# openai/procgen

Measured on NVIDIA H100. Metric: env-steps/sec, higher is better.
Workload: dtype f32+u8

## Files before the change

procgen_b200/csrc/pg_launch.cuh:

```cuda
#pragma once
#include <stdarg.h>
#include <stddef.h>
#include <stdio.h>
#include <stdlib.h>
#include <string.h>

#include <type_traits>

#include "pg_kernels.cuh"

#ifndef PG_HOSTSIM
#include <cuda_runtime.h>
#endif

namespace pg {

static inline void pg_fatal(const char *fmt, ...) {
    fprintf(stderr, "fatal: ");
    va_list args;
    va_start(args, fmt);
    vfprintf(stderr, fmt, args);
    va_end(args);
    exit(EXIT_FAILURE);
}
#define pg_fassert(cond)                                                                  \
    do {                                                                                  \
        if (!(cond)) {                                                                    \
            fprintf(stderr, "fassert failed '%s' at %s:%d\n", #cond, __FILE__, __LINE__); \
            exit(EXIT_FAILURE);                                                           \
        }                                                                                 \
    } while (0)

#ifndef PG_HOSTSIM
#define CUDA_CHECK(expr)                                                                          \
    do {                                                                                          \
        cudaError_t _e = (expr);                                                                  \
        if (_e != cudaSuccess)                                                                    \
            pg_fatal("CUDA error %s at %s:%d: %s\n", cudaGetErrorName(_e), __FILE__, __LINE__, cudaGetErrorString(_e)); \
    } while (0)
using Stream = cudaStream_t;
using Event = cudaEvent_t;
#else
struct HostStream;
struct HostEvent;
using Stream = HostStream *;
using Event = HostEvent *;
#endif

#ifndef PG_LOGIC_WARPS
#define PG_LOGIC_WARPS 2
#endif
#ifndef PG_LOGIC_MIN_BLOCKS
#define PG_LOGIC_MIN_BLOCKS 24
#endif
#ifndef PG_STEP_CHUNKS
#define PG_STEP_CHUNKS 8
#endif
#ifndef PG_AUX_STREAMS
#define PG_AUX_STREAMS 16
#endif
constexpr int kLogicThreads = 32 * PG_LOGIC_WARPS;
constexpr int kLogicEnvsPerBlock = PG_LOGIC_WARPS;
constexpr int kRenderThreads = 128;

#ifndef PG_HOSTSIM
template <class G, bool INIT, bool LEVEL_CHOICE = false, bool FINAL = false, bool PAUSE = false>
__global__ void __launch_bounds__(kLogicThreads, PG_LOGIC_MIN_BLOCKS) logic_kernel(KParams p, unsigned int *ticket) {
    using Frame = typename FrameFor<G>::type;
    const unsigned lane = threadIdx.x & 31u;
    while (true) {
        unsigned t = 0;
        if (lane == 0)
            t = atomicAdd(ticket, 1u);
        t = __shfl_sync(0xffffffffu, t, 0);
        if (t >= (unsigned)p.env_count)
            break;
        const int env = p.env_first + (int)t * p.env_step;
        const long long t0 = p.dbg_cycles ? clock64() : 0;
        env_logic<G, Frame, INIT, LEVEL_CHOICE, FINAL, PAUSE>(p, env);
        __syncwarp();
        if (p.dbg_cycles && lane == 0)
            p.dbg_cycles[env] = (uint32_t)(clock64() - t0);
    }
}

template <class G, bool BANK = false, bool LOOK = false>
__global__ void __launch_bounds__(kLogicThreads, PG_LOGIC_MIN_BLOCKS) finish_kernel(KParams p, unsigned int *ticket) {
    using Frame = typename FrameFor<G>::type;
    const unsigned lane = threadIdx.x & 31u;
    const unsigned count = *p.reset_count;
    while (true) {
        unsigned t = 0;
        if (lane == 0)
            t = atomicAdd(ticket, 1u);
        t = __shfl_sync(0xffffffffu, t, 0);
        if (t >= count)
            break;
        const int env = p.reset_list[t];
        const long long t0 = ((BANK || LOOK) && p.dbg_cycles) ? clock64() : 0;
        env_finish_logic<G, Frame, BANK, LOOK>(p, env);
        __syncwarp();
        if ((BANK || LOOK) && p.dbg_cycles && lane == 0)
            p.dbg_cycles[env] += (uint32_t)(clock64() - t0);
    }
}

template <class G>
__global__ void __launch_bounds__(kLogicThreads) bank_build_kernel(KParams p, unsigned char *stage, int count, int warps) {
    const int w = (int)((blockIdx.x * blockDim.x + threadIdx.x) >> 5);
    if (w >= warps)
        return;
    for (int item = w; item < count; item += warps) {
        bank_generate_level<G>(p, p.bank, p.bank.seeds[item], [&] { return p.bank.slots + (size_t)item * p.bank.slot_bytes; },
                               stage + (size_t)w * bank_stage_bytes(p));
        __syncwarp();
    }
}

template <class G>
__global__ void __launch_bounds__(kLogicThreads) lookahead_kernel(KParams p, unsigned int *count) {
    const int w = (int)((blockIdx.x * blockDim.x + threadIdx.x) >> 5);
    if (w >= p.look.stage_warps)
        return;
    const unsigned lane = threadIdx.x & 31u;
    const unsigned n = count[0];
    unsigned char *stage = p.look.stage + (size_t)w * bank_stage_bytes(p);
    while (true) {
        unsigned t = 0;
        if (lane == 0)
            t = atomicAdd(count + 1, 1u);
        t = __shfl_sync(0xffffffffu, t, 0);
        if (t >= n)
            break;
        lookahead_generate<G>(p, (int)t, stage);
        __syncwarp();
    }
}

template <class G>
__global__ void __launch_bounds__(kLogicThreads) lookahead_predict_kernel(KParams p) {
    const int i = (int)((blockIdx.x * blockDim.x + threadIdx.x) >> 5);
    if (i < p.env_count)
        lookahead_predict(p, p.env_first + i * p.env_step, p.bank.slots != nullptr);
}

constexpr int kSetupThreads = 128;
#ifndef PG_SETUP_MIN_BLOCKS
#define PG_SETUP_MIN_BLOCKS 8
#endif
template <class G, int VIEW>
struct SetupTune {
    static constexpr int kSmemBytes = (int)sizeof(typename FrameFor<G, VIEW>::setup) * (kSetupThreads / 32);
    static constexpr int kFit = (227 * 1024) / (kSmemBytes + 1024 + 128);
    static constexpr int kMinBlocks = kFit >= PG_SETUP_MIN_BLOCKS ? PG_SETUP_MIN_BLOCKS : (kFit >= 1 ? kFit : 1);
};
template <class G, int VIEW, bool LIST = false, bool PAUSE = false>
__global__ void __launch_bounds__(kSetupThreads, SetupTune<G, VIEW>::kMinBlocks) setup_kernel(KParams p) {
    using Setup = typename FrameFor<G, VIEW>::setup;
    extern __shared__ __align__(128) unsigned char smem_raw[];
    Setup &f = reinterpret_cast<Setup *>(smem_raw)[threadIdx.x >> 5];
    const int lane = (int)(threadIdx.x & 31u);
    const int i = (int)blockIdx.x * (kSetupThreads / 32) + (int)(threadIdx.x >> 5);
    if (LIST) {
        const int count = (int)*p.reset_count;
        for (int j = i; j < count; j += (int)gridDim.x * (kSetupThreads / 32)) {
            const int env = p.reset_list[j];
            env_setup_frame<G, Setup>(p, env, f, lane, 32);
            __syncwarp();
            PG_SETUP_PHASE_BEGIN;
            env_store_frame<Setup>(p, env, f);
            PG_SETUP_PHASE(9);
        }
        return;
    }
    if (i >= p.env_count)
        return;
    const int env = p.env_first + i * p.env_step;
    if (PAUSE && p.paused[env])
        return;
    env_setup_frame<G, Setup>(p, env, f, lane, 32);
    __syncwarp();
    PG_SETUP_PHASE_BEGIN;
    env_store_frame<Setup>(p, env, f);
    PG_SETUP_PHASE(9);
}

#ifndef PG_RENDER_CTAS_PER_SM
#define PG_RENDER_CTAS_PER_SM 0
#endif
template <class G, int VIEW>
struct RenderTune {
    static constexpr size_t kFrameBytes = sizeof(typename FrameFor<G, VIEW>::type);
#ifdef PG_RENDER_MIN_BLOCKS
    static constexpr int kMinBlocks = PG_RENDER_MIN_BLOCKS;
#else
    static constexpr int kFit = (int)((227 * 1024) / (kFrameBytes + 1024 + 16));
    static constexpr int kWant = G::DRAWS_GRID ? 7 : 8;
    static constexpr int kMinBlocks = kFit >= kWant ? kWant : (kFit >= 1 ? kFit : 1);
#endif
};

__device__ __forceinline__ uint32_t pg_smem_addr(const void *ptr) { return (uint32_t)__cvta_generic_to_shared(ptr); }
__device__ __forceinline__ void pg_mbar_init(unsigned long long *bar, unsigned count) {
    asm volatile("mbarrier.init.shared::cta.b64 [%0], %1;" ::"r"(pg_smem_addr(bar)), "r"(count) : "memory");
    asm volatile("fence.mbarrier_init.release.cluster;" ::: "memory");
}
__device__ __forceinline__ void pg_mbar_arrive_expect_tx(unsigned long long *bar, unsigned bytes) {
    asm volatile("mbarrier.arrive.expect_tx.shared::cta.b64 _, [%0], %1;" ::"r"(pg_smem_addr(bar)), "r"(bytes) : "memory");
}
__device__ __forceinline__ void pg_mbar_wait(unsigned long long *bar, unsigned parity) {
    unsigned done = 0;
    while (!done) {
        asm volatile(
            "{\n"
            ".reg .pred p;\n"
            "mbarrier.try_wait.parity.shared::cta.b64 p, [%1], %2;\n"
            "selp.u32 %0, 1, 0, p;\n"
            "}\n"
            : "=r"(done)
            : "r"(pg_smem_addr(bar)), "r"(parity)
            : "memory");
    }
}
__device__ __forceinline__ void pg_bulk_load(void *dst_smem, const void *src_gmem, unsigned bytes, unsigned long long *bar) {
    asm volatile("cp.async.bulk.shared::cluster.global.mbarrier::complete_tx::bytes [%0], [%1], %2, [%3];" ::"r"(pg_smem_addr(dst_smem)),
                 "l"(src_gmem), "r"(bytes), "r"(pg_smem_addr(bar))
                 : "memory");
}
__device__ __forceinline__ void pg_bulk_store(void *dst_gmem, const void *src_smem, unsigned bytes) {
    asm volatile("cp.async.bulk.global.shared::cta.bulk_group [%0], [%1], %2;" ::"l"(dst_gmem), "r"(pg_smem_addr(src_smem)), "r"(bytes) : "memory");
}
__device__ __forceinline__ void pg_bulk_commit_and_wait() {
    asm volatile("cp.async.bulk.commit_group;" ::: "memory");
    asm volatile("cp.async.bulk.wait_group.read 0;" ::: "memory");
}

template <class G, int VIEW, int PASS, bool ROLL, class EnvOf>
__device__ __forceinline__ void render_env_frame(const KParams &p, typename FrameFor<G, VIEW>::type &f, EnvOf env_of, unsigned parity) {
    using Frame = typename FrameFor<G, VIEW>::type;
    const int tid = (int)threadIdx.x;
#ifdef PG_PHASE_TIMING
    long long t0 = clock64(), t1;
#define PG_RENDER_PHASE(id)                                       \
    do {                                                          \
        t1 = clock64();                                           \
        if (tid == 0)                                             \
            p.hdr[env_of()].dbg_phase[id] = (uint32_t)(t1 - t0);       \
        t0 = t1;                                                  \
    } while (0)
#else
#define PG_RENDER_PHASE(id) do { } while (0)
#endif
    using Shared = typename FrameFor<G, VIEW>::shared;
    const Shared *gs = reinterpret_cast<const Shared *>(p.frame_setup + (size_t)env_of() * p.frame_setup_stride);
    if (tid < 32) {
        const int nj = G::DRAWS_GRID ? (gs->n_tjobs < MAX_TILE_JOBS ? gs->n_tjobs : MAX_TILE_JOBS) : 0;
        unsigned words = 0;
        for (int j = tid; j < nj; j += 32) words += gs->tjob_words[j];
        for (int d = 16; d > 0; d >>= 1) words += __shfl_xor_sync(0xffffffffu, words, d);
        if (tid == 0) {
            pg_mbar_arrive_expect_tx(&f.mbar, (unsigned)sizeof(Shared) + 4u * words);
            pg_bulk_load(static_cast<Shared *>(&f), gs, (unsigned)sizeof(Shared), &f.mbar);
        }
        __syncwarp();
        for (int j = tid; j < nj; j += 32)
            pg_bulk_load(f.arena + gs->tjob_dst[j], p.tiles.texels + gs->tjob_src[j], 4u * gs->tjob_words[j], &f.mbar);
    }
    pg_mbar_wait(&f.mbar, parity);
    PG_RENDER_PHASE(0);
    env_render_compose<G, Frame>(p, f, tid >> 5, kRenderThreads >> 5, tid & 31, 32);
    __syncthreads();
    PG_RENDER_PHASE(5);
    if (p.consumer != nullptr && !is_final_frame<PASS>(p, env_of())) {
        const int kf = p.consumer_k, s = *p.consumer_slot_dev;
        const int slots = kf == 1 ? 1 : 2 * kf;
        uint32_t *base = reinterpret_cast<uint32_t *>(p.consumer) + (size_t)env_of() * slots * (3 * RES_W * RES_H / 2);
        const uint16_t *lut = p.consumer_lut;
        for (int pair = tid; pair < RES_W * RES_H / 2; pair += kRenderThreads) {
            const uint32_t c0 = f.fb[2 * pair], c1 = f.fb[2 * pair + 1];
#pragma unroll
            for (int ch = 0; ch < 3; ch++) {
                const int sh = 16 - 8 * ch;
                const uint32_t v = (uint32_t)lut[(c0 >> sh) & 0xffu] | ((uint32_t)lut[(c1 >> sh) & 0xffu] << 16);
                base[(size_t)(s * 3 + ch) * (RES_W * RES_H / 2) + pair] = v;
                if (kf > 1)
                    base[(size_t)((s + kf) * 3 + ch) * (RES_W * RES_H / 2) + pair] = v;
            }
        }
        if (kf > 1 && p.first[env_of()]) {
            for (int j = 1; j < kf; j++) {
                const int a = (s + j) % kf;
                for (int w = tid; w < 3 * RES_W * RES_H / 2; w += kRenderThreads) {
                    base[(size_t)a * (3 * RES_W * RES_H / 2) + w] = 0u;
                    base[(size_t)(a + kf) * (3 * RES_W * RES_H / 2) + w] = 0u;
                }
            }
        }
    }
    {
        constexpr int kQuadsPerThread = RES_W * RES_H / 4 / kRenderThreads;
        uint32_t c[kQuadsPerThread][4];
#pragma unroll
        for (int j = 0; j < kQuadsPerThread; j++) {
            const uint4 v = reinterpret_cast<const uint4 *>(f.fb)[tid + j * kRenderThreads];
            c[j][0] = v.x; c[j][1] = v.y; c[j][2] = v.z; c[j][3] = v.w;
        }
        __syncthreads();
#pragma unroll
        for (int j = 0; j < kQuadsPerThread; j++) Raster<G, Frame>::pack_quad(c[j], f.fb + 3 * (tid + j * kRenderThreads));
    }
    asm volatile("fence.proxy.async.shared::cta;" ::: "memory");
    __syncthreads();
    PG_RENDER_PHASE(6);
    if (tid == 0) {
        pg_bulk_store((is_final_frame<PASS>(p, env_of()) ? p.final_rgb : p.rgb) + (size_t)env_of() * (RES_W * RES_H * 3), f.fb,
                      RES_W * RES_H * 3);
        if (ROLL && !is_final_frame<PASS>(p, env_of())) {
            pg_bulk_store(p.roll.rgb + rollout_index(p, env_of()) * (RES_W * RES_H * 3), f.fb, RES_W * RES_H * 3);
            rollout_store_scalars(p, env_of());
        }
        pg_bulk_commit_and_wait();
    }
    PG_RENDER_PHASE(7);
#undef PG_RENDER_PHASE
}

__device__ __forceinline__ void consumer_repeat_frame(const KParams &p, int env) {
    constexpr int kSlotVecs = 3 * RES_W * RES_H * 2 / 16;
    const int kf = p.consumer_k, s = *p.consumer_slot_dev;
    uint4 *base = reinterpret_cast<uint4 *>(p.consumer) + (size_t)env * (2 * kf) * kSlotVecs;
    const uint4 *src = base + (size_t)((s - 1 + kf) % kf) * kSlotVecs;
    for (int w = (int)threadIdx.x; w < kSlotVecs; w += kRenderThreads) {
        const uint4 v = src[w];
        base[(size_t)s * kSlotVecs + w] = v;
        base[(size_t)(s + kf) * kSlotVecs + w] = v;
    }
}

template <class G, int VIEW, int PASS = 0, bool PAUSE = false, bool ROLL = false>
__global__ void __launch_bounds__(kRenderThreads, RenderTune<G, VIEW>::kMinBlocks) render_kernel(KParams p) {
    static_assert(!(PAUSE && PASS == 2), "phase B's list never holds a paused env");
    using Frame = typename FrameFor<G, VIEW>::type;
    extern __shared__ __align__(128) unsigned char smem_raw[];
    Frame &f = *reinterpret_cast<Frame *>(smem_raw);
    if (PAUSE && p.paused[p.env_first + (int)blockIdx.x * p.env_step]) {
        if (p.consumer != nullptr && p.consumer_k > 1)
            consumer_repeat_frame(p, p.env_first + (int)blockIdx.x * p.env_step);
        if (ROLL)
            rollout_copy_frame(p, p.env_first + (int)blockIdx.x * p.env_step, (int)threadIdx.x, kRenderThreads);
        return;
    }
    if (threadIdx.x == 0)
        pg_mbar_init(&f.mbar, 1);
    __syncthreads();
    if (PASS == 2) {
        __shared__ int list_env;
        for (unsigned i = 0;; i++) {
            const int j = (int)(blockIdx.x + i * gridDim.x);
            if (j >= (int)*p.reset_count)
                break;
            if (threadIdx.x == 0)
                list_env = p.reset_list[j];
            __syncthreads();
            render_env_frame<G, VIEW, PASS, ROLL>(p, f, [&] { return list_env; }, i & 1u);
            __syncthreads();
        }
        return;
    }
    render_env_frame<G, VIEW, PASS, ROLL>(p, f, [&] { return p.env_first + (int)blockIdx.x * p.env_step; }, 0);
}

template <class G>
__global__ void camera_kernel(KParams p) {
    using Frame = typename FrameFor<G>::type;
    if (threadIdx.x == 0 && blockIdx.x < (unsigned)p.env_count)
        env_observe<G, Frame>(p, p.env_first + (int)blockIdx.x * p.env_step);
}

template <class G>
__global__ void camera_list_kernel(KParams p) {
    using Frame = typename FrameFor<G>::type;
    if (threadIdx.x == 0 && blockIdx.x < *p.reset_count)
        env_observe<G, Frame>(p, p.reset_list[blockIdx.x]);
}
#endif

template <class G, int VIEW, int PASS, bool ROLL>
void render_env_serial(const KParams &p, int env) {
    using Frame = typename FrameFor<G, VIEW>::type;
    using Setup = typename FrameFor<G, VIEW>::setup;
    using Shared = typename FrameFor<G, VIEW>::shared;
    static thread_local Frame *f = new Frame;
    static thread_local Setup *s = new Setup;
    memset(static_cast<void *>(s), 0xA5, sizeof(Setup));
    env_setup_frame<G, Setup>(p, env, *s, 0, 1);
    env_store_frame<Setup>(p, env, *s);
    static_cast<Shared &>(*f) = *reinterpret_cast<const Shared *>(p.frame_setup + (size_t)env * p.frame_setup_stride);
    env_stage_tiles_serial<Frame>(p, *f);
    for (int w = 0; w < 4; w++) env_render_compose<G, Frame>(p, *f, w, 4, 0, 1);
    const bool final_frame = is_final_frame<PASS>(p, env);
    uint8_t *rgb = final_frame ? p.final_rgb : p.rgb;
    uint32_t *out = reinterpret_cast<uint32_t *>(rgb + (size_t)env * (RES_W * RES_H * 3));
    for (int g = 0; g < RES_W * RES_H / 4; g++) Raster<G, Frame>::pack_quad(f->fb + 4 * g, out + 3 * g);
    if (ROLL && !final_frame)
        rollout_copy_frame(p, env, 0, 1);
}

struct alignas(32) TicketSlot {
    unsigned int logic;
    unsigned int reset_count;
    unsigned int finish;
    unsigned int look_count;
    unsigned int look;
};

struct StepShape {
    bool init = false;
    bool level_choice = false;
    bool pause = false;
    bool final_outputs = false;
    bool bank = false;
    bool look = false;
    bool roll = false;
    bool two_phase() const { return final_outputs || bank || look; }
    size_t ticket_bytes() const {
        return look ? offsetof(TicketSlot, look) + sizeof(unsigned int)
                    : two_phase() ? offsetof(TicketSlot, finish) + sizeof(unsigned int) : sizeof(unsigned int);
    }
};

struct LaunchCtx {
    Stream stream;
    Stream logic_stream;
    Event link;
    int max_logic_blocks;
    int num_sms;
    int render_smem_floor;
    Event *tev;
    TicketSlot *ticket;
    Stream look_stream;
    Event look_fork;
    int64_t *launch_counter;
};

template <class F>
void with_flag(bool flag, F &&f) {
    if (flag)
        f(std::true_type{});
    else
        f(std::false_type{});
}

#ifndef PG_HOSTSIM
template <auto K>
int dynamic_smem(int bytes) {
    static int attr_set[64] = {};
    int dev = 0;
    CUDA_CHECK(cudaGetDevice(&dev));
    int &have = attr_set[dev & 63];
    if (have < bytes) {
        CUDA_CHECK(cudaFuncSetAttribute(K, cudaFuncAttributeMaxDynamicSharedMemorySize, bytes));
        have = bytes;
    }
    return bytes;
}

static inline int logic_grid(const KParams &p, const LaunchCtx &lc) {
    const int blocks = (p.env_count + kLogicEnvsPerBlock - 1) / kLogicEnvsPerBlock;
    return blocks < lc.max_logic_blocks ? blocks : lc.max_logic_blocks;
}
#endif


template <class G, bool INIT, bool LEVEL_CHOICE, bool FINAL, bool PAUSE>
void logic_kernels(const KParams &p, const LaunchCtx &lc, size_t ticket_bytes) {
#ifndef PG_HOSTSIM
    const cudaStream_t ls = !FINAL && lc.logic_stream ? lc.logic_stream : lc.stream;
    CUDA_CHECK(cudaMemsetAsync(lc.ticket, 0, ticket_bytes, ls));
    if (lc.tev)
        CUDA_CHECK(cudaEventRecord(lc.tev[0], ls));
    logic_kernel<G, INIT, LEVEL_CHOICE, FINAL, PAUSE><<<logic_grid(p, lc), kLogicThreads, 0, ls>>>(p, &lc.ticket->logic);
    CUDA_CHECK(cudaGetLastError());
    if (ls != lc.stream) {
        CUDA_CHECK(cudaEventRecord(lc.link, ls));
        CUDA_CHECK(cudaStreamWaitEvent(lc.stream, lc.link, 0));
    }
#else
    using Frame = typename FrameFor<G>::type;
    memset(lc.ticket, 0, ticket_bytes);
    for (int i = 0; i < p.env_count; i++) env_logic<G, Frame, INIT, LEVEL_CHOICE, FINAL, PAUSE>(p, p.env_first + i * p.env_step);
#endif
    (*lc.launch_counter) += 1;
}

template <class G>
void logic_phase(const KParams &p, const LaunchCtx &lc, const StepShape &s) {
    if (s.init)
        return logic_kernels<G, true, false, false, false>(p, lc, s.ticket_bytes());
    with_flag(s.pause, [&](auto pause) {
        with_flag(s.two_phase(), [&](auto final) {
            if constexpr (final)
                logic_kernels<G, false, false, true, pause>(p, lc, s.ticket_bytes());
            else
                with_flag(s.level_choice, [&](auto choice) { logic_kernels<G, false, choice, false, pause>(p, lc, s.ticket_bytes()); });
        });
    });
}

template <class G>
void finish_phase(const KParams &p, const LaunchCtx &lc, const StepShape &s) {
    with_flag(s.bank, [&](auto bank) {
        with_flag(s.look, [&](auto look) {
#ifndef PG_HOSTSIM
            finish_kernel<G, bank, look><<<logic_grid(p, lc), kLogicThreads, 0, lc.stream>>>(p, &lc.ticket->finish);
            CUDA_CHECK(cudaGetLastError());
#else
            using Frame = typename FrameFor<G>::type;
            for (unsigned int j = 0; j < *p.reset_count; j++) env_finish_logic<G, Frame, bank, look>(p, p.reset_list[j]);
#endif
        });
    });
    (*lc.launch_counter) += 1;
}

template <class G>
void lookahead_phase(const KParams &p, const LaunchCtx &lc) {
#ifndef PG_HOSTSIM
    CUDA_CHECK(cudaEventRecord(lc.look_fork, lc.stream));
    CUDA_CHECK(cudaStreamWaitEvent(lc.look_stream, lc.look_fork, 0));
    const int blocks = (p.look.stage_warps + kLogicEnvsPerBlock - 1) / kLogicEnvsPerBlock;
    lookahead_kernel<G><<<blocks, kLogicThreads, 0, lc.look_stream>>>(p, p.look.count);
    CUDA_CHECK(cudaGetLastError());
#else
    for (unsigned int j = 0; j < *p.look.count; j++) lookahead_generate<G>(p, (int)j, p.look.stage);
#endif
    (*lc.launch_counter) += 1;
}

template <class G, int VIEW, int PASS, bool PAUSE, bool ROLL>
void frames_kernels(const KParams &p, const LaunchCtx &lc) {
    constexpr bool LIST = PASS == 2;
#ifndef PG_HOSTSIM
    using Frame = typename FrameFor<G, VIEW>::type;
    const int setup_smem = dynamic_smem<setup_kernel<G, VIEW, LIST, PAUSE>>(SetupTune<G, VIEW>::kSmemBytes);
    const int render_smem = dynamic_smem<render_kernel<G, VIEW, PASS, PAUSE, ROLL>>(
        (int)sizeof(Frame) > lc.render_smem_floor ? (int)sizeof(Frame) : lc.render_smem_floor);
    int setup_blocks = (p.env_count + kSetupThreads / 32 - 1) / (kSetupThreads / 32);
    int render_blocks = p.env_count;
    if (LIST) {
        const int setup_fit = lc.num_sms * SetupTune<G, VIEW>::kMinBlocks, render_fit = lc.num_sms * RenderTune<G, VIEW>::kMinBlocks;
        setup_blocks = setup_blocks < setup_fit ? setup_blocks : setup_fit;
        render_blocks = render_blocks < render_fit ? render_blocks : render_fit;
    }
    if (lc.tev)
        CUDA_CHECK(cudaEventRecord(lc.tev[1], lc.stream));
    setup_kernel<G, VIEW, LIST, PAUSE><<<setup_blocks, kSetupThreads, setup_smem, lc.stream>>>(p);
    if (lc.tev)
        CUDA_CHECK(cudaEventRecord(lc.tev[2], lc.stream));
    render_kernel<G, VIEW, PASS, PAUSE, ROLL><<<render_blocks, kRenderThreads, render_smem, lc.stream>>>(p);
    if (lc.tev)
        CUDA_CHECK(cudaEventRecord(lc.tev[3], lc.stream));
    CUDA_CHECK(cudaGetLastError());
#else
    (void)lc;
    if (LIST) {
        for (unsigned int j = 0; j < *p.reset_count; j++) render_env_serial<G, VIEW, PASS, ROLL>(p, p.reset_list[j]);
    } else {
        for (int i = 0; i < p.env_count; i++) {
            const int env = p.env_first + i * p.env_step;
            if (!(PAUSE && p.paused[env]))
                render_env_serial<G, VIEW, PASS, ROLL>(p, env);
            else if (ROLL)
                rollout_copy_frame(p, env, 0, 1);
        }
    }
#endif
    (*lc.launch_counter) += 2;
}

template <class G, int VIEW, int PASS>
void frames_phase(const KParams &p, const LaunchCtx &lc, const StepShape &s) {
    with_flag(s.roll, [&](auto roll) {
        if constexpr (PASS == 2)
            frames_kernels<G, VIEW, PASS, false, roll>(p, lc);
        else
            with_flag(s.pause, [&](auto pause) { frames_kernels<G, VIEW, PASS, pause, roll>(p, lc); });
    });
}

template <class G, int VIEW>
void launch_step(const KParams &p, const LaunchCtx &lc, const StepShape &s) {
    if (p.env_count <= 0)
        return;
    if (!s.two_phase()) {
        logic_phase<G>(p, lc, s);
        frames_phase<G, VIEW, 0>(p, lc, s);
        return;
    }
    KParams q = p;
    q.reset_count = &lc.ticket->reset_count;
    q.look.count = &lc.ticket->look_count;
    if (!s.final_outputs)
        q.level_end = p.bank_level_end;
    logic_phase<G>(q, lc, s);
    if (s.final_outputs)
        frames_phase<G, VIEW, 1>(q, lc, s);
    finish_phase<G>(q, lc, s);
    if (s.look)
        lookahead_phase<G>(q, lc);
    if (s.final_outputs)
        frames_phase<G, VIEW, 2>(q, lc, s);
    else
        frames_phase<G, VIEW, 0>(p, lc, s);
}

template <class G, int VIEW>
void launch_observe_only(const KParams &p, const LaunchCtx &lc) {
    if (p.env_count <= 0)
        return;
#ifndef PG_HOSTSIM
    camera_kernel<G><<<p.env_count, 32, 0, lc.stream>>>(p);
    CUDA_CHECK(cudaGetLastError());
#else
    using Frame = typename FrameFor<G>::type;
    for (int i = 0; i < p.env_count; i++) env_observe<G, Frame>(p, p.env_first + i * p.env_step);
#endif
    frames_phase<G, VIEW, 0>(p, lc, StepShape{});
}

template <class G, int VIEW>
void launch_observe_list(const KParams &p, const LaunchCtx &lc) {
    if (p.env_count <= 0)
        return;
#ifndef PG_HOSTSIM
    camera_list_kernel<G><<<p.env_count, 32, 0, lc.stream>>>(p);
    CUDA_CHECK(cudaGetLastError());
#else
    using Frame = typename FrameFor<G>::type;
    for (unsigned int j = 0; j < *p.reset_count; j++) env_observe<G, Frame>(p, p.reset_list[j]);
#endif
    frames_phase<G, VIEW, 2>(p, lc, StepShape{});
}

template <class G>
void launch_bank_build(const KParams &p, const LaunchCtx &lc, unsigned char *stage, int warps, int count) {
    if (count <= 0)
        return;
#ifndef PG_HOSTSIM
    const int blocks = (warps + kLogicEnvsPerBlock - 1) / kLogicEnvsPerBlock;
    bank_build_kernel<G><<<blocks, kLogicThreads, 0, lc.stream>>>(p, stage, count, warps);
    CUDA_CHECK(cudaGetLastError());
    (*lc.launch_counter) += 1;
#else
    (void)lc;
    (void)warps;
    for (int item = 0; item < count; item++)
        bank_generate_level<G>(p, p.bank, p.bank.seeds[item], [&] { return p.bank.slots + (size_t)item * p.bank.slot_bytes; }, stage);
#endif
}

template <class G>
void launch_lookahead_fill(const KParams &p, const LaunchCtx &lc) {
    if (p.env_count <= 0)
        return;
#ifndef PG_HOSTSIM
    lookahead_predict_kernel<G><<<(p.env_count + kLogicEnvsPerBlock - 1) / kLogicEnvsPerBlock, kLogicThreads, 0, lc.stream>>>(p);
    CUDA_CHECK(cudaGetLastError());
    const int blocks = (p.look.stage_warps + kLogicEnvsPerBlock - 1) / kLogicEnvsPerBlock;
    lookahead_kernel<G><<<blocks, kLogicThreads, 0, lc.stream>>>(p, p.look.count);
    CUDA_CHECK(cudaGetLastError());
    (*lc.launch_counter) += 2;
#else
// ... 62 lines not shown
```

procgen_b200/csrc/pg_raster.cuh:

```cuda
#pragma once
#include "pg_engine.cuh"

namespace pg {

enum BlitKind : uint8_t { BLIT_NONE = 0, BLIT_IMAGE = 1, BLIT_SOLID = 2, BLIT_ROTATED = 3, BLIT_SPANS = 4,
                          BLIT_ROT_PENDING = 5  };

struct Blit {
    uint8_t x1, y1, w, h;
    uint8_t kind;
    uint8_t mirror;
    uint16_t opacity;
    int32_t ix, iy;
    uint32_t basex, srcy;
    uint32_t src;
    uint16_t sw, sh;
};
static_assert(sizeof(Blit) == 32, "Blit is 32 B");

struct RotBlit {
    uint8_t x1[RES_H], x2[RES_H];
    int32_t absolute;
    int32_t dudx, dvdx, dudy, dvdy, u0, v0;
    int32_t pad;
// ... 1396 lines not shown
                                f.job_ei[job] = ei;
                                f.job_pos[job] = pos;
                                f.job_n[job] = mine;
                                f.job_j0[job] = entity_first_visible_tile(c, f, ei);
                            } else
#endif
                            {
                                Blit *dst = f.ents + pos;
                                entity_blits(c, f, ei, true, single, [=](int j, const Blit &b) { dst[j] = b; });
                            }
                        }
                    } else {
                        c.h->err |= ERR_ENT_BLITS;
                    }
                }
                count += total;
#if defined(__CUDA_ARCH__)
                if (multi_warp)
                    __syncthreads();
#endif
            }
            if (z == -1)
                below = count;
        }
        if (count > Frame::kMaxEntBlits)
            count = Frame::kMaxEntBlits;
        if (below > count)
            below = count;
        if (tid == 0) {
            if (!G::ENTS_BELOW_GRID && below > 0)
                c.h->err |= ERR_UNSUPPORTED;
            f.n_ent = count;
            f.n_ent_below = below;
            if (count > c.h->max_blits_seen)
                c.h->max_blits_seen = count;
            if (f.n_rot > c.h->max_rots_seen)
                c.h->max_rots_seen = f.n_rot;
        }
    }

    static PG_HD bool clipped_walk_matches(int s, int t, int k0) {
        if (k0 == 0)
            return true;
        const double sx = (double)s / (double)t;
        const int ix = (int)(65536.0 * sx);
        const uint32_t bu = (uint32_t)((int)pg_dceil((0 + 0.5 - 0.0) * sx * 65536) - 1);
        const uint32_t bc = (uint32_t)((int)pg_dceil((0 + 0.5 - (double)(-k0)) * sx * 65536) - 1);
        for (int j = 0; j + k0 < t; j++)
            if (((bc + (uint32_t)ix * (uint32_t)j) >> 16) != ((bu + (uint32_t)ix * (uint32_t)(j + k0)) >> 16))
                return false;
        return true;
    }

    static PG_HD void frame_build(Ctx &c, Frame &f, int tid, int nthreads, int ) {
        const int wtid = tid, wn = nthreads;
        if (f.pad == 1) {
            const Blit &b = f.bg[0];
            for (int py = wtid; py < RES_H; py += wn) {
                const uint32_t dy = (uint32_t)py - b.y1;
                f.bgrow[py] = dy < b.h ? b.src + ((b.srcy + (uint32_t)b.iy * dy) >> 16) * b.sw : BG_NONE;
            }
        }
        if (!G::DRAWS_GRID)
            return;
        for (int px = wtid; px < RES_W + RES_H; px += wn) {
            if (px < RES_W) {
                const uint32_t w = cell_lookup(f.col_p1, f.col_p2, f.col_tw, f.col_k0, f.nx, f.ny, px, f.col_lo[px], f.col_hi[px]);
                f.colinfo[px] = w;
                if (w & CI_MULTI) {
                    int slot;
#if defined(__CUDA_ARCH__)
                    slot = atomicAdd(&f.n_strip_cols, 1);
#else
                    slot = f.n_strip_cols++;
#endif
                    f.strip_cols[slot] = (uint8_t)px;
                }
            } else {
                f.rowinfo[px - RES_W] = cell_lookup(f.row_p1, f.row_p2, f.row_th, f.row_k0, f.ny, 1, px - RES_W, f.row_lo[px - RES_W], f.row_hi[px - RES_W]);
            }
        }
        const int ncells = f.nx * f.ny;
        const bool mono = c.h->options.use_monochrome_assets != 0;
#if defined(__CUDA_ARCH__)
        for (int j = wtid; j < f.ny; j += wn) {
            const int gy = f.low_y + j, gx = f.low_x < 0 ? 0 : f.low_x;
            if (gy >= 0 && gy < c.mh && gx < c.mw) {
                const int16_t *row = c.grid + gy * c.mw + gx;
                asm volatile("prefetch.global.L1 [%0];" ::"l"(row));
                if (f.nx > 32 || ((reinterpret_cast<uintptr_t>(row) & 127) + 2 * f.nx > 128))
                    asm volatile("prefetch.global.L1 [%0];" ::"l"(row + f.nx - 1 < c.grid + c.mh * c.mw ? row + f.nx - 1 : row));
            }
        }
#endif
        int ci = f.ny > 0 ? wtid / f.ny : 0, cj = wtid - ci * f.ny;
        for (int k = wtid; k < ncells; k += wn) {
            if (k != wtid) {
                cj += wn;
                while (cj >= f.ny) {
                    cj -= f.ny;
                    ci++;
                }
            }
            f.cellmap[k] = 0;
            if (f.col_p1[ci] >= f.col_p2[ci] || f.row_p1[cj] >= f.row_p2[cj])
                continue;
            int type = E::get_obj(c, f.low_x + ci, f.low_y + cj);
            if (type == INVALID_OBJ)
                continue;
            const int img_type = G::image_for_type(c, type);
            if (img_type < 0 || img_type == SPACE)
                continue;
            const int theme = G::theme_for_grid_obj(c, type);
            const int tw = f.col_tw[ci], th = f.row_th[cj];
            if (tw && th && !mono && type >= 0 && type < CELL_KEY_TYPES && theme >= 0 && theme < MAX_IMAGE_THEMES) {
                double adj[4];
                bool ok = img_type >= 0 && img_type < USE_ASSET_THRESHOLD && !G::get_adjusted_image_rect(c, img_type, adj);
                if (ok && (f.col_k0[ci] | f.row_k0[cj])) {
                    const int masked_theme = (c.h->options.restrict_themes && !G::should_preserve_type_themes(c, img_type)) ? 0 : theme;
                    const SpriteDesc sd = c.assets->sprites[img_type + masked_theme * MAX_ASSETS];
                    ok = sd.w != 0 && clipped_walk_matches(sd.w, tw, f.col_k0[ci]) && clipped_walk_matches(sd.h, th, f.row_k0[cj]);
                }
                if (ok) {
                    const int key = type * 4 + (tw - f.tile_w0) + 2 * (th - f.tile_h0);
                    f.tilekey[key] = 1;
                    f.cellmap[k] = (uint16_t)(0x4000 | key);
                    continue;
                }
            }
            int slot;
#if defined(__CUDA_ARCH__)
            slot = atomicAdd(&f.n_gen, 1);
#else
            slot = f.n_gen++;
#endif
            Blit b;
            double r[4] = {f.col_x[ci], f.row_y[cj], f.cell_w, f.cell_w};
            make_sprite_blit(c, f, b, r, 0, false, type, theme, 1.0f);
            if (b.kind == BLIT_NONE)
                continue;
            *f.gen_blit(slot) = b;
            f.cellmap[k] = (uint16_t)(CELL_GENERAL | slot);
        }
    }

    static PG_HD void frame_tile_alloc(Ctx &c, Frame &f, const TileTable &tt, int tid, int nthreads) {
        if (!G::DRAWS_GRID)
            return;
        for (int key = tid; key < CELL_KEYS; key += nthreads) {
            if (f.tilekey[key] != 1)
                continue;
            const int type = key >> 2;
            const int tw = f.tile_w0 + (key & 1), th = f.tile_h0 + ((key >> 1) & 1);
            const int img_type = G::image_for_type(c, type);
            const int theme = G::theme_for_grid_obj(c, type);
            const int masked_theme = (c.h->options.restrict_themes && !G::should_preserve_type_themes(c, img_type)) ? 0 : theme;
            const int slot = tt.texels ? c.assets->sprite_slot[img_type + masked_theme * MAX_ASSETS] : -1;
            uint16_t code = 0xffffu;
            if (slot >= 0) {
                const int words = tile_words(tw, th);
                int off, job;
#if defined(__CUDA_ARCH__)
                off = atomicAdd(&f.tile_top, words);
#else
                off = f.tile_top;
                f.tile_top += words;
#endif
                if (off + words <= Frame::kArenaWords) {
#if defined(__CUDA_ARCH__)
                    job = atomicAdd(&f.n_tjobs, 1);
#else
                    job = f.n_tjobs++;
#endif
                    if (job < MAX_TILE_JOBS) {
                        f.tjob_src[job] = tt.index[(slot * MAX_TILE_DIM + (tw - 1)) * MAX_TILE_DIM + (th - 1)];
                        f.tjob_dst[job] = (uint16_t)off;
                        f.tjob_words[job] = (uint16_t)words;
                        code = (uint16_t)(2 + off);
                    }
                }
            }
            f.tilekey[key] = code;
        }
    }

    static PG_HD void frame_cells_finish(Ctx &c, Frame &f, int tid, int nthreads) {
        if (!G::DRAWS_GRID)
            return;
        const int ncells = f.nx * f.ny;
        for (int k = tid; k < ncells; k += nthreads) {
            const uint16_t code = f.cellmap[k];
            if ((code & 0xC000u) != 0x4000u)
                continue;
            const int key = code & 0x3fff;
            const uint16_t tk = f.tilekey[key];
            if (tk != 0xffffu) {
                f.cellmap[k] = (uint16_t)(tk - 1);
                continue;
            }
            f.cellmap[k] = 0;
            int slot;
#if defined(__CUDA_ARCH__)
            slot = atomicAdd(&f.n_gen, 1);
#else
            slot = f.n_gen++;
#endif
            const int ci = k / f.ny, cj = k - ci * f.ny;
            const int type = key >> 2;
            Blit b;
            double r[4] = {f.col_x[ci], f.row_y[cj], f.cell_w, f.cell_w};
            make_sprite_blit(c, f, b, r, 0, false, type, G::theme_for_grid_obj(c, type), 1.0f);
            if (b.kind == BLIT_NONE)
                continue;
            *f.gen_blit(slot) = b;
            f.cellmap[k] = (uint16_t)(CELL_GENERAL | slot);
        }
    }

    static PG_HD void frame_tiles(Ctx &c, Frame &f, int tid, int nthreads) {
        const int nj = f.n_jobs < Frame::kMaxTileJobs ? f.n_jobs : Frame::kMaxTileJobs;
        for (int job = 0; job < nj; job++) {
            const int ei = f.job_ei[job], pos = f.job_pos[job], nt = f.job_n[job], j0 = f.job_j0[job];
            for (int j = tid; j < nt; j += nthreads) entity_tile_blit(c, f, ei, j0 + j, f.ents[pos + j]);
        }
    }

    static PG_HD void frame_rots(Ctx &c, Frame &f, int tid, int nthreads) {
        const int n = f.n_ent;
        for (int i = tid; i < n; i += nthreads) {
            if (f.ents[i].kind != BLIT_ROT_PENDING)
                continue;
            const int ei = (int)f.ents[i].src;
            const Entity &o = c.ents[ei];
            double r[4];
            object_rect(f.cam, o, r);
            Blit nb;
            make_sprite_blit(c, f, nb, r, o.rotation, o.is_reflected != 0, o.image_type, o.image_theme, o.alpha);
            f.ents[i] = nb;
        }
    }

    static PG_HD void frame_append_overlays(Frame &f) {
        for (int i = 0; i < f.n_overlay; i++) f.ents[f.n_ent + i] = f.overlay[i];
    }

    static PG_HD int ctz64(uint64_t m) {
#if defined(__CUDA_ARCH__)
        return __ffsll((long long)m) - 1;
#else
        return __builtin_ctzll(m);
#endif
    }
    static PG_HD int top_bit64(uint64_t m) {
#if defined(__CUDA_ARCH__)
        return 63 - __clzll((long long)m);
#else
        return 63 - __builtin_clzll(m);
#endif
    }


    static PG_HD uint32_t cell_layer(const Frame &f, uint32_t code, int ci, int cj, int px, int py, const uint32_t *atlas) {
        if (code & CELL_GENERAL)
            return blit_texel(*f.gen_blit((int)(code & 0x7fffu)), px, py, atlas, f.rot);
        const int dx = px - f.col_p1[ci] + f.col_k0[ci], dy = py - f.row_p1[cj] + f.row_k0[cj];
        return f.arena[(int)code - 1 + dy * f.col_tw[ci] + dx];
    }

    static PG_HD uint32_t bg_column(const Frame &f, int px) {
        const Blit &b = f.bg[0];
        const uint32_t dx = (uint32_t)px - b.x1;
        return dx < b.w ? (b.basex + (uint32_t)b.ix * dx) >> 16 : BG_NONE;
    }
    static PG_HD uint32_t bg_single(uint32_t bgrow, uint32_t bgcol, const uint32_t *atlas) {
        return (bgrow != BG_NONE && bgcol != BG_NONE) ? atlas[bgrow + bgcol] : 0xff000000u;
    }
    static PG_HD_NOINLINE uint32_t bg_generic(const Frame &f, int px, int py, const uint32_t *atlas) {
        uint32_t dst = 0xff000000u;
        if (f.pad == 1)
            return bg_single(f.bgrow[py], bg_column(f, px), atlas);
        for (int i = 0; i < f.n_bg; i++) dst = layer_over(dst, blit_texel(f.bg[i], px, py, atlas, f.rot));
        return dst;
    }

    static PG_HD uint32_t cells_over(const Frame &f, int px, int py, const uint32_t *atlas, uint32_t under) {
        uint32_t dst = under;
        const int clo = f.col_lo[px], chi = f.col_hi[px], rlo = f.row_lo[py], rhi = f.row_hi[py];
        if (clo != 255 && rlo != 255) {
            for (int ci = clo; ci <= chi; ci++)
                for (int cj = rlo; cj <= rhi; cj++) {
                    const uint32_t code = f.cellmap[ci * f.ny + cj];
                    if (code && px >= f.col_p1[ci] && px < f.col_p2[ci] && py >= f.row_p1[cj] && py < f.row_p2[cj])
                        dst = layer_over(dst, cell_layer(f, code, ci, cj, px, py, atlas));
                }
        }
        return dst;
    }
    static PG_HD_NOINLINE uint32_t cells_generic(const Frame &f, int px, int py, const uint32_t *atlas, uint32_t under) {
        return cells_over(f, px, py, atlas, under);
    }

    struct QuadCtx {
        uint32_t ci[4];
        uint32_t cbase[4];
        uint32_t tile_dx[4], tile_tw[4];
        uint32_t bg_sx[4];
        bool bg_one;
    };
    static PG_HD void quad_begin(const Frame &f, int px0, QuadCtx &q) {
        q.bg_one = f.pad == 1;
        for (int k = 0; k < 4; k++) {
            const uint32_t ci = G::DRAWS_GRID ? f.colinfo[px0 + k] : 0u;
            q.ci[k] = ci;
            q.cbase[k] = ci & CI_BASE_MASK;
            q.tile_dx[k] = (ci >> CI_D_SHIFT) & 31u;
            q.tile_tw[k] = (ci >> CI_TW_SHIFT) & 31u;
            q.bg_sx[k] = q.bg_one ? bg_column(f, px0 + k) : 0u;
        }
    }

    enum GatherMode { GATHER_ALL = 0, GATHER_BG = 1, GATHER_CELLS = 2 };

    template <int MODE>
    static PG_HD void gather_quad(const Frame &f, const QuadCtx &q, int px0, int py, const uint32_t *atlas, uint32_t *fb) {
        const uint32_t rowinfo = (G::DRAWS_GRID && MODE != GATHER_BG) ? f.rowinfo[py] : 0u;
        const uint32_t bgrow = q.bg_one ? f.bgrow[py] : BG_NONE;
        const uint32_t rbase = rowinfo & CI_BASE_MASK, dy = (rowinfo >> CI_D_SHIFT) & 31u;
        uint32_t *dst = fb + py * RES_W + px0;
        uint32_t s[4];
        uint32_t slow = 0, strip = 0;
        for (int k = 0; k < 4; k++) {
            s[k] = 0;
            if (G::DRAWS_GRID && MODE != GATHER_BG) {
                const uint32_t both = q.ci[k] & rowinfo;
                if (both & CI_FAST) {
                    const uint32_t code = f.cellmap[q.cbase[k] + rbase];
                    if (code & CELL_GENERAL) {
                        const Blit &gb = *f.gen_blit((int)(code & 0x7fffu));
                        if (gb.kind == BLIT_SOLID) {
                            const uint32_t box = *reinterpret_cast<const uint32_t *>(&gb);
                            const uint32_t ddx = (uint32_t)(px0 + k) - (box & 0xffu), ddy = (uint32_t)py - ((box >> 8) & 0xffu);
                            s[k] = (ddx < ((box >> 16) & 0xffu) && ddy < (box >> 24)) ? gb.src : 0u;
                        } else {
                            slow |= 1u << k;
                        }
                    } else if (code) {
                        s[k] = f.arena[code - 1 + dy * q.tile_tw[k] + q.tile_dx[k]];
                    }
                } else if (both & CI_VALID) {
                    strip |= 1u << k;
                }
            }
        }
        uint32_t c[4];
        for (int k = 0; k < 4; k++) {
            c[k] = s[k];
            if ((strip >> k) & 1u)
                continue;
            if (s[k] >= 0xff000000u && !((slow >> k) & 1u))
                continue;
            uint32_t under;
            if (MODE == GATHER_CELLS)
                under = dst[k];
            else if (q.bg_one)
                under = bg_single(bgrow, q.bg_sx[k], atlas);
            else
                under = bg_generic(f, px0 + k, py, atlas);
            if ((slow >> k) & 1u)
                c[k] = cells_generic(f, px0 + k, py, atlas, under);
            else
                c[k] = s[k] != 0 ? s[k] + pg_byte_mul(under, (~s[k]) >> 24) : under;
        }
        if (MODE == GATHER_CELLS) {
            for (int k = 0; k < 4; k++)
                if (!((strip >> k) & 1u))
                    dst[k] = c[k];
        } else {
#if defined(__CUDA_ARCH__)
            *reinterpret_cast<uint4 *>(dst) = make_uint4(c[0], c[1], c[2], c[3]);
#else
            for (int k = 0; k < 4; k++) dst[k] = c[k];
#endif
        }
    }

    template <int MODE>
    static PG_HD void gather_strips(const Frame &f, uint32_t *fb, int row_first, int row_step, int lane, int nlanes, const uint32_t *atlas) {
        const int my_rows = (RES_H - row_first + row_step - 1) / row_step;
        const int n1 = f.n_strip_cols * my_rows;
        for (int idx = lane; idx < n1; idx += nlanes) {
            const int px = f.strip_cols[idx / my_rows], py = row_first + (idx % my_rows) * row_step;
            if (!(f.rowinfo[py] & CI_VALID))
                continue;
            uint32_t *dst = fb + py * RES_W + px;
            const uint32_t under = MODE == GATHER_CELLS ? *dst : bg_generic(f, px, py, atlas);
            *dst = cells_over(f, px, py, atlas, under);
        }
        for (int r = 0; r < my_rows; r++) {
            const int py = row_first + r * row_step;
            if (!(f.rowinfo[py] & CI_MULTI))
                continue;
            for (int px = lane; px < RES_W; px += nlanes) {
                const uint32_t ci = f.colinfo[px];
                if (!(ci & CI_VALID) || (ci & CI_MULTI))
                    continue;
                uint32_t *dst = fb + py * RES_W + px;
                const uint32_t under = MODE == GATHER_CELLS ? *dst : bg_generic(f, px, py, atlas);
                *dst = cells_over(f, px, py, atlas, under);
            }
        }
    }

    static PG_HD void paint_blits(const Frame &f, uint32_t *fb, int lo, int hi, int row_first, int row_step, int lane, int nlanes, const uint32_t *atlas) {
        for (int i = lo; i < hi; i++) {
            const Blit &b = f.ents[i];
            const uint32_t box = *reinterpret_cast<const uint32_t *>(&b);
            const int x1 = (int)(box & 0xffu), y1 = (int)((box >> 8) & 0xffu), w = (int)((box >> 16) & 0xffu), h = (int)(box >> 24);
            if (w == 0)
                continue;
            int r0 = (row_first - y1) % row_step;
            if (r0 < 0)
                r0 += row_step;
            const int nrows = r0 < h ? (h - 1 - r0) / row_step + 1 : 0;
            const int n = nrows * w;
            const bool plain = b.kind == BLIT_IMAGE;
            for (int idx = lane; idx < n; idx += nlanes) {
                const int r = idx / w, dx = idx - r * w, dy = r0 + r * row_step;
                uint32_t s;
                if (plain) {
                    uint32_t sx = (b.basex + (uint32_t)b.ix * (uint32_t)dx) >> 16;
                    const uint32_t sy = (b.srcy + (uint32_t)b.iy * (uint32_t)dy) >> 16;
                    if (b.mirror)
                        sx = b.sw - 1 - sx;
                    s = layer_of(atlas[b.src + sy * b.sw + sx], b.opacity);
                } else {
                    s = blit_texel(b, x1 + dx, y1 + dy, atlas, f.rot);
                }
                if (s != 0) {
                    uint32_t *px = fb + (y1 + dy) * RES_W + x1 + dx;
                    *px = layer_over(*px, s);
                }
            }
#if defined(__CUDA_ARCH__)
            __syncwarp();
#endif
        }
    }

    static PG_HD void pack_quad(const uint32_t *c, uint32_t *out) {
#if defined(__CUDA_ARCH__)
        out[0] = __byte_perm(c[0], c[1], 0x6012);
        out[1] = __byte_perm(c[1], c[2], 0x5601);
        out[2] = __byte_perm(c[2], c[3], 0x4560);
#else
        const uint32_t r0 = (c[0] >> 16) & 0xff, g0 = (c[0] >> 8) & 0xff, b0 = c[0] & 0xff;
        const uint32_t r1 = (c[1] >> 16) & 0xff, g1 = (c[1] >> 8) & 0xff, b1 = c[1] & 0xff;
        const uint32_t r2 = (c[2] >> 16) & 0xff, g2 = (c[2] >> 8) & 0xff, b2 = c[2] & 0xff;
        const uint32_t r3 = (c[3] >> 16) & 0xff, g3 = (c[3] >> 8) & 0xff, b3 = c[3] & 0xff;
        out[0] = r0 | (g0 << 8) | (b0 << 16) | (r1 << 24);
        out[1] = g1 | (b1 << 8) | (r2 << 16) | (g2 << 24);
        out[2] = b2 | (r3 << 8) | (g3 << 16) | (b3 << 24);
#endif
    }

    static PG_HD void compose_rows(const Frame &f, uint32_t *fb, int row_first, int row_step, int lane, int nlanes, const uint32_t *atlas) {
        const int nb = f.n_ent_below, n_all = f.n_ent + f.n_overlay;
        const int per_row = RES_W / 4;
        const int sub = nlanes >= per_row ? nlanes / per_row : 1;
        for (int qx = lane % per_row; qx < per_row; qx += (nlanes < per_row ? nlanes : per_row)) {
            QuadCtx q;
            quad_begin(f, qx * 4, q);
            const int first = row_first + row_step * (nlanes >= per_row ? lane / per_row : 0);
            if (G::ENTS_BELOW_GRID && nb > 0) {
                for (int py = first; py < RES_H; py += row_step * sub) gather_quad<GATHER_BG>(f, q, qx * 4, py, atlas, fb);
            } else {
                for (int py = first; py < RES_H; py += row_step * sub) gather_quad<GATHER_ALL>(f, q, qx * 4, py, atlas, fb);
            }
        }
        if (G::DRAWS_GRID && !(G::ENTS_BELOW_GRID && nb > 0))
            gather_strips<GATHER_ALL>(f, fb, row_first, row_step, lane, nlanes, atlas);
        if (G::ENTS_BELOW_GRID && nb > 0) {
#if defined(__CUDA_ARCH__)
            __syncwarp();
#endif
            paint_blits(f, fb, 0, nb, row_first, row_step, lane, nlanes, atlas);
            for (int qx = lane % per_row; qx < per_row; qx += (nlanes < per_row ? nlanes : per_row)) {
                QuadCtx q;
                quad_begin(f, qx * 4, q);
                const int first = row_first + row_step * (nlanes >= per_row ? lane / per_row : 0);
                for (int py = first; py < RES_H; py += row_step * sub) gather_quad<GATHER_CELLS>(f, q, qx * 4, py, atlas, fb);
            }
            if (G::DRAWS_GRID)
                gather_strips<GATHER_CELLS>(f, fb, row_first, row_step, lane, nlanes, atlas);
        }
#if defined(__CUDA_ARCH__)
        __syncwarp();
#endif
        paint_blits(f, fb, (G::ENTS_BELOW_GRID ? nb : 0), n_all, row_first, row_step, lane, nlanes, atlas);
    }
};

template <class G>
struct DrawDefaults {
    template <class Frame>
    static PG_HD void make_background_blits(Ctx &c, Frame &f) {
        EnvHdr &h = *c.h;
        double main_rect[4];
        Raster<G, Frame>::screen_rect(f.cam, 0, (float)h.main_height, (float)h.main_width, (float)h.main_height, 0, main_rect);
        SpriteDesc bg = c.assets->backgrounds[h.background_index];
        if (h.bg_tile_ratio < 0) {
            const int nt = Raster<G, Frame>::tile_count(main_rect, h.bg_tile_ratio);
            int n = 0;
            for (int i = 0; i < nt; i++) {
                double tr[4];
                Raster<G, Frame>::tile_rect(main_rect, h.bg_tile_ratio, nt, i, tr);
                Blit b;
                make_image_blit(b, tr[0], tr[1], tr[2], tr[3], bg, false, 256, f.snap != 0);
                if (b.kind == BLIT_NONE)
                    continue;
                if (n < MAX_BG_BLITS)
                    f.bg[n++] = b;
                else
                    h.err |= ERR_BLIT_OVERFLOW;
            }
            f.n_bg = n;
            return;
        }
        float bgw = bg.w;
        float bgh = bg.h;
        float bg_ar = bgw / bgh;
        float world_ar = (float)(h.main_width * 1.0 / h.main_height);
        float extra_w = bg_ar - world_ar;
        float offset_x = h.bg_pct_x * extra_w;
        double adj[4] = {(double)(-offset_x), 0, (double)(bg_ar / world_ar), 1};
        Raster<G, Frame>::adjust_rect(main_rect, adj);
        make_image_blit(f.bg[0], main_rect[0], main_rect[1], main_rect[2], main_rect[3], bg, false, 256, f.snap != 0);
        f.n_bg = 1;
    }
    template <class Frame>
    static PG_HD void make_overlay_blits(Ctx &c, Frame &f) {}
    template <class Frame>
    static PG_HD bool make_grid_obj_blit(Ctx &c, const Frame &f, Blit &b, double *rect, int type, int theme) {
        if (!c.h->options.use_monochrome_assets)
            return false;
        if (c.h->options.restrict_themes && !G::should_preserve_type_themes(c, type))
            theme = 0;
        const int k = 4;
        const int kcubed = k * k * k;
        const int chunk = 256 / k;
        if (type >= kcubed)
            return false;
        int new_type = (29 * (type + 1)) % kcubed;
        new_type = (new_type + 19 * theme) % kcubed;
        const uint32_t r = (uint32_t)(chunk * (new_type / (k * k) + 1) - 1);
        const uint32_t g = (uint32_t)(chunk * ((new_type / k) % k + 1) - 1);
        const uint32_t bl = (uint32_t)(chunk * (new_type % k + 1) - 1);
        make_solid_blit(b, rect[0], rect[1], rect[2], rect[3], (r << 16) | (g << 8) | bl);
        return true;
    }
};

}
```

Before: 22.09 million.

## Cut render kernel register pressure and issue tile bulk loads before summing sizes

The quad context no longer caches decoded per-column fields and decodes them from colinfo at use. Entity counts for grid games are reloaded late rather than held in registers, the block index is read through inline PTX, and the reset-list loop counter is kept in shared memory. Together these aim to lower register use so grid games can run 8 CTAs per SM instead of 7. Tile bulk copies are now issued right away, with the mbarrier byte count added through expect_tx before the final arrive, so the separate pass that summed tile sizes before loading is gone. The cost is extra bit decoding in the inner gather and a dependence on MAX_TILE_JOBS being exactly 64.

```diff
diff --git a/procgen_b200/csrc/pg_launch.cuh b/procgen_b200/csrc/pg_launch.cuh
--- a/procgen_b200/csrc/pg_launch.cuh
+++ b/procgen_b200/csrc/pg_launch.cuh
@@ -195,10 +195,16 @@
     static constexpr int kMinBlocks = PG_RENDER_MIN_BLOCKS;
 #else
     static constexpr int kFit = (int)((227 * 1024) / (kFrameBytes + 1024 + 16));
-    static constexpr int kWant = G::DRAWS_GRID ? 7 : 8;
+    static constexpr int kWant = G::DRAWS_GRID && G::ENTS_BELOW_GRID ? 7 : 8;
     static constexpr int kMinBlocks = kFit >= kWant ? kWant : (kFit >= 1 ? kFit : 1);
 #endif
 };
+
+__device__ __forceinline__ unsigned pg_cta_x() {
+    unsigned x;
+    asm volatile("mov.u32 %0, %%ctaid.x;" : "=r"(x));
+    return x;
+}
 
 __device__ __forceinline__ uint32_t pg_smem_addr(const void *ptr) { return (uint32_t)__cvta_generic_to_shared(ptr); }
 __device__ __forceinline__ void pg_mbar_init(unsigned long long *bar, unsigned count) {
@@ -207,6 +213,9 @@
 }
 __device__ __forceinline__ void pg_mbar_arrive_expect_tx(unsigned long long *bar, unsigned bytes) {
     asm volatile("mbarrier.arrive.expect_tx.shared::cta.b64 _, [%0], %1;" ::"r"(pg_smem_addr(bar)), "r"(bytes) : "memory");
+}
+__device__ __forceinline__ void pg_mbar_expect_tx(unsigned long long *bar, unsigned bytes) {
+    asm volatile("mbarrier.expect_tx.relaxed.cta.shared::cta.b64 [%0], %1;" ::"r"(pg_smem_addr(bar)), "r"(bytes) : "memory");
 }
 __device__ __forceinline__ void pg_mbar_wait(unsigned long long *bar, unsigned parity) {
     unsigned done = 0;
@@ -254,17 +263,30 @@
     using Shared = typename FrameFor<G, VIEW>::shared;
     const Shared *gs = reinterpret_cast<const Shared *>(p.frame_setup + (size_t)env_of() * p.frame_setup_stride);
     if (tid < 32) {
-        const int nj = G::DRAWS_GRID ? (gs->n_tjobs < MAX_TILE_JOBS ? gs->n_tjobs : MAX_TILE_JOBS) : 0;
+        if (tid == 0) {
+            pg_mbar_expect_tx(&f.mbar, (unsigned)sizeof(Shared));
+            pg_bulk_load(static_cast<Shared *>(&f), gs, (unsigned)sizeof(Shared), &f.mbar);
+        }
         unsigned words = 0;
-        for (int j = tid; j < nj; j += 32) words += gs->tjob_words[j];
-        for (int d = 16; d > 0; d >>= 1) words += __shfl_xor_sync(0xffffffffu, words, d);
-        if (tid == 0) {
-            pg_mbar_arrive_expect_tx(&f.mbar, (unsigned)sizeof(Shared) + 4u * words);
-            pg_bulk_load(static_cast<Shared *>(&f), gs, (unsigned)sizeof(Shared), &f.mbar);
-        }
-        __syncwarp();
-        for (int j = tid; j < nj; j += 32)
-            pg_bulk_load(f.arena + gs->tjob_dst[j], p.tiles.texels + gs->tjob_src[j], 4u * gs->tjob_words[j], &f.mbar);
+        if (G::DRAWS_GRID) {
+            static_assert(MAX_TILE_JOBS == 64, "two tile jobs per lane");
+            const int n = gs->n_tjobs;
+            const int nj = n < MAX_TILE_JOBS ? n : MAX_TILE_JOBS;
+            const uint32_t src0 = gs->tjob_src[tid], src1 = gs->tjob_src[tid + 32];
+            const unsigned dst0 = gs->tjob_dst[tid], dst1 = gs->tjob_dst[tid + 32];
+            const unsigned w0 = gs->tjob_words[tid], w1 = gs->tjob_words[tid + 32];
+            if (tid < nj) {
+                pg_bulk_load(f.arena + dst0, p.tiles.texels + src0, 4u * w0, &f.mbar);
+                words += w0;
+            }
+            if (tid + 32 < nj) {
+                pg_bulk_load(f.arena + dst1, p.tiles.texels + src1, 4u * w1, &f.mbar);
+                words += w1;
+            }
+            for (int d = 16; d > 0; d >>= 1) words += __shfl_xor_sync(0xffffffffu, words, d);
+        }
+        if (tid == 0)
+            pg_mbar_arrive_expect_tx(&f.mbar, 4u * words);
     }
     pg_mbar_wait(&f.mbar, parity);
     PG_RENDER_PHASE(0);
@@ -355,7 +377,12 @@
     __syncthreads();
     if (PASS == 2) {
         __shared__ int list_env;
-        for (unsigned i = 0;; i++) {
+        __shared__ unsigned list_round;
+        if (threadIdx.x == 0)
+            list_round = 0;
+        __syncthreads();
+        while (true) {
+            const unsigned i = list_round;
             const int j = (int)(blockIdx.x + i * gridDim.x);
             if (j >= (int)*p.reset_count)
                 break;
@@ -363,11 +390,13 @@
                 list_env = p.reset_list[j];
             __syncthreads();
             render_env_frame<G, VIEW, PASS, ROLL>(p, f, [&] { return list_env; }, i & 1u);
+            if (threadIdx.x == 0)
+                list_round += 1;
             __syncthreads();
         }
         return;
     }
-    render_env_frame<G, VIEW, PASS, ROLL>(p, f, [&] { return p.env_first + (int)blockIdx.x * p.env_step; }, 0);
+    render_env_frame<G, VIEW, PASS, ROLL>(p, f, [&] { return p.env_first + (int)(G::DRAWS_GRID ? pg_cta_x() : blockIdx.x) * p.env_step; }, 0);
 }
 
 template <class G>
diff --git a/procgen_b200/csrc/pg_raster.cuh b/procgen_b200/csrc/pg_raster.cuh
--- a/procgen_b200/csrc/pg_raster.cuh
+++ b/procgen_b200/csrc/pg_raster.cuh
@@ -1722,19 +1722,13 @@
 
     struct QuadCtx {
         uint32_t ci[4];
-        uint32_t cbase[4];
-        uint32_t tile_dx[4], tile_tw[4];
         uint32_t bg_sx[4];
         bool bg_one;
     };
     static PG_HD void quad_begin(const Frame &f, int px0, QuadCtx &q) {
         q.bg_one = f.pad == 1;
         for (int k = 0; k < 4; k++) {
-            const uint32_t ci = G::DRAWS_GRID ? f.colinfo[px0 + k] : 0u;
-            q.ci[k] = ci;
-            q.cbase[k] = ci & CI_BASE_MASK;
-            q.tile_dx[k] = (ci >> CI_D_SHIFT) & 31u;
-            q.tile_tw[k] = (ci >> CI_TW_SHIFT) & 31u;
+            q.ci[k] = G::DRAWS_GRID ? f.colinfo[px0 + k] : 0u;
             q.bg_sx[k] = q.bg_one ? bg_column(f, px0 + k) : 0u;
         }
     }
@@ -1754,7 +1748,7 @@
             if (G::DRAWS_GRID && MODE != GATHER_BG) {
                 const uint32_t both = q.ci[k] & rowinfo;
                 if (both & CI_FAST) {
-                    const uint32_t code = f.cellmap[q.cbase[k] + rbase];
+                    const uint32_t code = f.cellmap[(q.ci[k] & CI_BASE_MASK) + rbase];
                     if (code & CELL_GENERAL) {
                         const Blit &gb = *f.gen_blit((int)(code & 0x7fffu));
                         if (gb.kind == BLIT_SOLID) {
@@ -1765,7 +1759,7 @@
                             slow |= 1u << k;
                         }
                     } else if (code) {
-                        s[k] = f.arena[code - 1 + dy * q.tile_tw[k] + q.tile_dx[k]];
+                        s[k] = f.arena[code - 1 + dy * ((q.ci[k] >> CI_TW_SHIFT) & 31u) + ((q.ci[k] >> CI_D_SHIFT) & 31u)];
                     }
                 } else if (both & CI_VALID) {
                     strip |= 1u << k;
@@ -1884,7 +1878,8 @@
     }
 
     static PG_HD void compose_rows(const Frame &f, uint32_t *fb, int row_first, int row_step, int lane, int nlanes, const uint32_t *atlas) {
-        const int nb = f.n_ent_below, n_all = f.n_ent + f.n_overlay;
+        const int nb = G::ENTS_BELOW_GRID ? f.n_ent_below : 0;
+        const int n_all_held = G::DRAWS_GRID ? 0 : f.n_ent + f.n_overlay;
         const int per_row = RES_W / 4;
         const int sub = nlanes >= per_row ? nlanes / per_row : 1;
         for (int qx = lane % per_row; qx < per_row; qx += (nlanes < per_row ? nlanes : per_row)) {
@@ -1916,7 +1911,8 @@
 #if defined(__CUDA_ARCH__)
         __syncwarp();
 #endif
-        paint_blits(f, fb, (G::ENTS_BELOW_GRID ? nb : 0), n_all, row_first, row_step, lane, nlanes, atlas);
+        paint_blits(f, fb, (G::ENTS_BELOW_GRID ? f.n_ent_below : 0), G::DRAWS_GRID ? f.n_ent + f.n_overlay : n_all_held, row_first,
+                    row_step, lane, nlanes, atlas);
     }
 };
 
```

After: 22.81 million, median of 6. 1.03x the previous value.
